# CPJKU/beat_this

Measured on AMD Instinct MI355X. Metric: audio-seconds processed/sec, higher is better.
Workload: dtype f32 activations, f16x3 products (3 x f16 MFMA on hi+lo operand halves, f32 accumulate); main-layer attention P.V: 2 x, probabilities as fp16 hi parts

## Files before the change

### beat_this_amd/csrc/gemm3.hip

```cpp
#include <cstdlib>

#include "common.h"
#include "kernels.h"

struct G3CfgS { static constexpr int BM = 128, BN = 128, BK = 32, WGM = 2, WGN = 2, NST = 3, OCC = 3; };
struct G3CfgB { static constexpr int BM = 256, BN = 256, BK = 64, WGM = 2, WGN = 4, NST = 2, OCC = 1; };
struct G3CfgT { static constexpr int BM = 192, BN = 256, BK = 64, WGM = 2, WGN = 4, NST = 2, OCC = 1; };
struct G3CfgSX { static constexpr int BM = 128, BN = 128, BK = 64, WGM = 2, WGN = 2, NST = 2, OCC = 2; };
struct G3CfgBX { static constexpr int BM = 256, BN = 256, BK = 64, WGM = 2, WGN = 4, NST = 2, OCC = 1; };
struct G3CfgTX { static constexpr int BM = 192, BN = 256, BK = 64, WGM = 2, WGN = 4, NST = 2, OCC = 1; };
struct G3CfgMX { static constexpr int BM = 256, BN = 128, BK = 32, WGM = 2, WGN = 2, NST = 3, OCC = 2; };
struct G3CfgHX { static constexpr int BM = 64, BN = 128, BK = 64, WGM = 2, WGN = 2, NST = 3, OCC = 2; };

#ifndef X3_NSPLIT
#define X3_NSPLIT 2
#endif

namespace {

typedef G3CfgS CfgS;
typedef G3CfgB CfgB;

constexpr unsigned OOB = 0x80000000u;

#ifndef BT_NT_STORE
#define BT_NT_STORE 1
#endif
#if BT_NT_STORE
#define ST_STREAM(ptr, val) __builtin_nontemporal_store((val), (ptr))
#else
#define ST_STREAM(ptr, val) (*(ptr) = (val))
#endif

typedef __amdgpu_buffer_rsrc_t rsrc_t;
typedef __attribute__((address_space(3))) void* lptr_t;
typedef __attribute__((ext_vector_type(4))) unsigned int u32x4;
typedef __attribute__((ext_vector_type(2))) unsigned int u32x2;

DEVI unsigned pk2(float a, float b) {
  const hfx2 t = {(hf)a, (hf)b};
  return __builtin_bit_cast(unsigned, t);
}

DEVI void pack_row_hf(const float (&v)[16], u32x4 (&piece)[2]) {
#pragma unroll
  for (int k = 0; k < 2; ++k) {
    unsigned x0 = pk2(v[8 * k], v[8 * k + 1]), x1 = pk2(v[8 * k + 2], v[8 * k + 3]);
    unsigned y0 = pk2(v[8 * k + 4], v[8 * k + 5]), y1 = pk2(v[8 * k + 6], v[8 * k + 7]);
    auto r0 = __builtin_amdgcn_permlane32_swap(x0, y0, false, false);
    auto r1 = __builtin_amdgcn_permlane32_swap(x1, y1, false, false);
    piece[k] = u32x4{r0[0], r1[0], r0[1], r1[1]};
  }
}

DEVI void split2(float a, float b, unsigned& whi, unsigned& wlo, float& amax) {
  split_hl(a, b, whi, wlo);
  amax = fmaxf(amax, fmaxf(fabsf(a), fabsf(b)));
}
DEVI void pack_row_hl(const float (&v)[16], u32x4 (&hi)[2], u32x4 (&lo)[2], float& amax) {
#pragma unroll
  for (int k = 0; k < 2; ++k) {
    unsigned xh[2], xl[2], yh[2], yl[2];
    split2(v[8 * k], v[8 * k + 1], xh[0], xl[0], amax);
    split2(v[8 * k + 2], v[8 * k + 3], xh[1], xl[1], amax);
    split2(v[8 * k + 4], v[8 * k + 5], yh[0], yl[0], amax);
    split2(v[8 * k + 6], v[8 * k + 7], yh[1], yl[1], amax);
    auto h0 = __builtin_amdgcn_permlane32_swap(xh[0], yh[0], false, false);
    auto h1 = __builtin_amdgcn_permlane32_swap(xh[1], yh[1], false, false);
    auto l0 = __builtin_amdgcn_permlane32_swap(xl[0], yl[0], false, false);
    auto l1 = __builtin_amdgcn_permlane32_swap(xl[1], yl[1], false, false);
    hi[k] = u32x4{h0[0], h1[0], h0[1], h1[1]};
    lo[k] = u32x4{l0[0], l1[0], l0[1], l1[1]};
  }
}
DEVI void pack_row_f8(const float (&v)[16], u32x4 (&hi)[2], u32x2 (&h8)[2], u32x2 (&l8)[2], float& amax) {
#pragma unroll
  for (int k = 0; k < 2; ++k) {
    unsigned xh[2], xl[2], yh[2], yl[2];
    split2(v[8 * k], v[8 * k + 1], xh[0], xl[0], amax);
    split2(v[8 * k + 2], v[8 * k + 3], xh[1], xl[1], amax);
    split2(v[8 * k + 4], v[8 * k + 5], yh[0], yl[0], amax);
    split2(v[8 * k + 6], v[8 * k + 7], yh[1], yl[1], amax);
    const unsigned x8 = pk4_f8(v[8 * k], v[8 * k + 1], v[8 * k + 2], v[8 * k + 3]);
    const unsigned y8 = pk4_f8(v[8 * k + 4], v[8 * k + 5], v[8 * k + 6], v[8 * k + 7]);
    const unsigned xl8 = lo4_f8(v[8 * k], v[8 * k + 1], v[8 * k + 2], v[8 * k + 3], xh[0], xh[1]);
    const unsigned yl8 = lo4_f8(v[8 * k + 4], v[8 * k + 5], v[8 * k + 6], v[8 * k + 7], yh[0], yh[1]);
    auto h0 = __builtin_amdgcn_permlane32_swap(xh[0], yh[0], false, false);
    auto h1 = __builtin_amdgcn_permlane32_swap(xh[1], yh[1], false, false);
    auto b8 = __builtin_amdgcn_permlane32_swap(x8, y8, false, false);
    auto c8 = __builtin_amdgcn_permlane32_swap(xl8, yl8, false, false);
    hi[k] = u32x4{h0[0], h1[0], h0[1], h1[1]};
    h8[k] = u32x2{b8[0], b8[1]};
    l8[k] = u32x2{c8[0], c8[1]};
  }
}
DEVI void flag_range(int* status, float amax, float limit = 65504.f) {
  if (status && __any(!(amax <= limit)) && (threadIdx.x & 63) == 0) atomicOr(status, 1);
}

template <int EPI, typename CFG, int X3 = 0, int ABL = 0>
__global__ __launch_bounds__(64 * CFG::WGM * CFG::WGN, (CFG::OCC * CFG::WGM * CFG::WGN + 3) / 4)
void gemm3_kernel(const Gemm3P p, int n_tiles, int total_tiles, int per_xcd, int nsplit) {
  constexpr int BM = CFG::BM, BN = CFG::BN, BK = CFG::BK, NST = CFG::NST;
  constexpr int NW = CFG::WGM * CFG::WGN, NT = 64 * NW;
  constexpr int TB = BM / CFG::WGM / 32;
  constexpr int FB = BN / CFG::WGN / 32;
  constexpr int ROWB = BK * 2;
  constexpr int KR = X3 ? BK / 2 : BK;
  constexpr bool HL16 = X3 && BK == 32;
  constexpr int EB = X3 ? 4 : 2;
  constexpr int CPR = ROWB / 16;
  constexpr int RPI = 64 / CPR;
  constexpr int A_BYTES = BM * ROWB, W_BYTES = BN * ROWB, ST_BYTES = A_BYTES + W_BYTES;
  constexpr int APC = A_BYTES / (NT * 16), WPC = W_BYTES / (NT * 16);
  static_assert(EPI != G3_QKV || TB == FB, "the V columns swap the operand roles: square wave tile needed");
  static_assert(BN / CFG::WGN == 64, "ssq partials are per 64 columns = one wave");
  static_assert(!X3 || ROWB == 128 || ROWB == 64, "hl32: a k-step is a whole group (128 B per row) or half of one (64 B)");
  static_assert(X3 != 2 || ROWB == 128, "hl8: a k-step is a whole 32-column group");
  static_assert(NST * ST_BYTES >= NW * 8192, "the epilogues stage 8 KB per wave in the ring's LDS");
  __shared__ __attribute__((aligned(16))) char smem[NST * ST_BYTES];
  const int bid = blockIdx.x;
  int m_tile, n_tile;
  if (nsplit <= 1) {
    const int tile = (bid & 7) * per_xcd + (bid >> 3);
    if (tile >= total_tiles) return;
    m_tile = tile / n_tiles;
    n_tile = tile - m_tile * n_tiles;
  } else {
    const int xcd = bid & 7, slot = bid >> 3;
    const int g = xcd % nsplit, j = xcd / nsplit, per_m = 8 / nsplit, nt = n_tiles / nsplit;
    const int m_local = slot / nt;
    m_tile = m_local * per_m + j;
    n_tile = g * nt + (slot - m_local * nt);
    if ((long)m_tile * n_tiles >= total_tiles) return;
  }
  const int m0 = m_tile * BM, n0 = n_tile * BN;
  const int tid = threadIdx.x, lane = tid & 63, wave = __builtin_amdgcn_readfirstlane(tid >> 6);
  const int g = lane >> 5, lr = lane & 31;
  const int wm = wave / CFG::WGN, wn = wave % CFG::WGN;
  const int nk = p.K / KR;
  auto swz = [](int r) { return ROWB == 64 ? (r >> 2) & 3 : (r >> 1) & 7; };
  const int Lv = p.nblk * 32;

  int kind = 0;
  if constexpr (EPI == G3_QKV) kind = n0 < 3 * p.inner ? n0 / p.inner : 3;
  const bool normal = EPI == G3_QKV && kind == 2;

  const unsigned a_bytes = (unsigned)((long)p.M * p.lda * EB), w_bytes = (unsigned)((long)n_tiles * BN * p.K * EB);
  static_assert(APC >= 1 && WPC >= 1, "tile too small for the workgroup");
  static_assert(APC <= 4 && WPC <= 4, "voffA / voffW hold at most 4 pieces");
  unsigned voffA[4], voffW[4];
  int tapmask[4] = {0, 0, 0, 0};
#pragma unroll
  for (int i = 0; i < APC; ++i) {
    const int r = (i * NW + wave) * RPI + lane / CPR;
    const int c = (lane % CPR) ^ swz(r);
    long row = (long)m0 + r;
    bool ok = row < p.M;
    if constexpr (EPI == G3_QKV) {
      const int seq = (int)(row / Lv), t = (int)(row - (long)seq * Lv);
      ok = seq < p.n_seq && t < p.L;
      row = (long)seq * p.L + t;
    }
#ifdef BT_ABL_HID_WRAP
    if (EPI == G3_RESID && X3 && p.K >= 1024 && p.conv_C2 == 0) row &= BT_ABL_HID_WRAP - 1;
#endif
    voffA[i] = ok ? (unsigned)(row * p.lda * EB + (HL16 ? (c >> 1) * 64 + (c & 1) * 16 : c * 16)) : OOB;
    if constexpr (EPI == G3_RESID) {
      const int t = p.conv_C2 > 0 ? (int)((row / p.conv_F) % p.conv_T) : 1;
      tapmask[i] = ok ? ((t >= 1 ? 1 : 0) | 2 | (t + 1 < p.conv_T ? 4 : 0)) : 0;
    }
  }
#pragma unroll
  for (int i = 0; i < WPC; ++i) {
    const int r = (i * NW + wave) * RPI + lane / CPR;
    const int c = (lane % CPR) ^ swz(r);
    voffW[i] = (unsigned)((long)(n0 + r) * p.K * EB + (HL16 ? (c >> 1) * 64 + (c & 1) * 16 : c * 16));
  }
  const bool conv = EPI == G3_RESID && p.conv_C2 > 0;
  const unsigned tap_bytes = conv ? (unsigned)(p.conv_F * p.conv_C2 * EB) : 0u;
  const int c2_shift = conv ? __builtin_ctz((unsigned)p.conv_C2) : 0;
  const rsrc_t rA = __builtin_amdgcn_make_buffer_rsrc(const_cast<char*>(reinterpret_cast<const char*>(p.A)) - tap_bytes, 0,
                                                      a_bytes + 2 * tap_bytes, 0x00020000);
  const rsrc_t rW = __builtin_amdgcn_make_buffer_rsrc(const_cast<void*>(p.W), 0, w_bytes, 0x00020000);
#define G3_ISSUE(kt, stage)                                                                                          \
  do {                                                                                                                \
    char* st_ = smem + (stage) * ST_BYTES + wave * 1024;                                                              \
    const int so_ = HL16 ? ((kt) >> 1) * 128 + ((kt) & 1) * 32 : (kt) * ROWB;                                         \
    if (conv) {                                                                                                       \
      const int tap_ = ((kt) * KR) >> c2_shift;                                                                       \
      const int kin_ = ((kt) * KR) & (p.conv_C2 - 1);                                                                 \
      const int soa_ = tap_ * (int)tap_bytes + (HL16 ? (kin_ >> 5) * 128 + ((kin_ >> 4) & 1) * 32 : kin_ * EB);      \
      _Pragma("unroll") for (int i_ = 0; i_ < APC; ++i_)                                                              \
          __builtin_amdgcn_raw_ptr_buffer_load_lds(rA, (lptr_t)(st_ + i_ * NW * 1024), 16,                            \
                                                   ((tapmask[i_] >> tap_) & 1) ? voffA[i_] : OOB, soa_, 0, 0);        \
    } else {                                                                                                          \
      _Pragma("unroll") for (int i_ = 0; i_ < APC; ++i_)                                                              \
          __builtin_amdgcn_raw_ptr_buffer_load_lds(rA, (lptr_t)(st_ + i_ * NW * 1024), 16, voffA[i_], so_, 0, 0);     \
    }                                                                                                                 \
    _Pragma("unroll") for (int i_ = 0; i_ < WPC; ++i_)                                                                \
        __builtin_amdgcn_raw_ptr_buffer_load_lds(rW, (lptr_t)(st_ + A_BYTES + i_ * NW * 1024), 16, voffW[i_], so_, 0, 0); \
  } while (0)

  constexpr int NP = FB, NQ = TB;
  const int pofs = (normal ? wm * (TB * 32) * ROWB : A_BYTES + wn * (FB * 32) * ROWB) + lr * ROWB;
  const int qofs = (normal ? A_BYTES + wn * (FB * 32) * ROWB : wm * (TB * 32) * ROWB) + lr * ROWB;
  const int sw = swz(lr);
  constexpr int MS = ROWB / 32;
  int kc[MS];
#pragma unroll
  for (int m = 0; m < MS; ++m) kc[m] = ((2 * m + g) ^ sw) * 16;

  f32x16 acc[NP][NQ];
#pragma unroll
  for (int a = 0; a < NP; ++a)
#pragma unroll
    for (int b = 0; b < NQ; ++b)
#pragma unroll
      for (int r = 0; r < 16; ++r) acc[a][b][r] = 0.f;

  const int row0 = m0 + wm * (TB * 32);
  long trow[TB];
  int tseq[TB], tblk[TB];
#pragma unroll
  for (int j = 0; j < TB; ++j) {
    const long v = (long)row0 + 32 * j + lr;
    if constexpr (EPI == G3_QKV) {
      const int vb = row0 + 32 * j;
      tseq[j] = vb / Lv;
      tblk[j] = (vb - tseq[j] * Lv) >> 5;
      const int t = tblk[j] * 32 + lr;
      trow[j] = (tseq[j] < p.n_seq && t < p.L) ? (long)tseq[j] * p.L + t : -1;
    } else {
      tseq[j] = tblk[j] = 0;
      trow[j] = v < p.M ? v : -1;
    }
  }
  float rs[TB], part[TB][8];
#pragma unroll
  for (int j = 0; j < TB; ++j) {
    rs[j] = 1.f;
#pragma unroll
    for (int q = 0; q < 8; ++q)
      part[j][q] = (EPI != G3_RESID && p.ssq_in && trow[j] >= 0 && q < p.ssq_parts) ? p.ssq_in[(long)q * p.M + trow[j]] : 0.f;
  }
  f32x4 bqv[EPI == G3_FF1 ? FB : 1][4];
  if constexpr (EPI == G3_FF1) {
#pragma unroll
    for (int a = 0; a < FB; ++a)
#pragma unroll
      for (int q = 0; q < 4; ++q) bqv[a][q] = *reinterpret_cast<const f32x4*>(p.bias + n0 + wn * 64 + a * 32 + 8 * q + 4 * g);
  }
  f32x4 csv[EPI == G3_QKV ? TB : 1][4];
  if constexpr (EPI == G3_QKV) {
    if (kind < 2) {
#pragma unroll
      for (int b = 0; b < TB; ++b)
#pragma unroll
        for (int q = 0; q < 4; ++q)
          csv[b][q] = tseq[b] < p.n_seq ? *reinterpret_cast<const f32x4*>(p.rope + ((long)(tblk[b] * 32 + lr) * 16 + 4 * q + 2 * g) * 2)
                                        : f32x4{0.f, 0.f, 0.f, 0.f};
    }
  }
  constexpr int LPS = APC + WPC;
#pragma unroll
  for (int s0 = 0; s0 < NST - 1; ++s0)
    if (s0 < nk) G3_ISSUE(s0, s0);
  if (EPI == G3_FF1 || EPI == G3_QKV || (EPI != G3_RESID && p.ssq_in)) {
    asm volatile("s_waitcnt vmcnt(0)" ::: "memory");
    __builtin_amdgcn_sched_barrier(0);
  }
  if (EPI != G3_RESID && p.ssq_in) {
#pragma unroll
    for (int j = 0; j < TB; ++j) {
      float sum = 0.f;
#pragma unroll
      for (int q = 0; q < 8; ++q) sum += part[j][q];
      for (int q = 8; q < p.ssq_parts; ++q) sum += trow[j] >= 0 ? p.ssq_in[(long)q * p.M + trow[j]] : 0.f;
      rs[j] = trow[j] >= 0 ? sqrtf((float)p.K) / fmaxf(sqrtf(sum), 1e-12f) : 0.f;
    }
  }
  int stage = 0, stage2 = NST - 1;
  long long t_wait = 0, t_bar = 0, t_loop0 = 0;
  if constexpr ((ABL & 8) != 0) t_loop0 = clock64();
  for (int kt = 0; kt < nk; ++kt) {
    long long tq0 = 0, tq1 = 0;
    if constexpr ((ABL & 8) != 0) tq0 = clock64();
    if (NST > 2 && kt + 1 < nk && !(ABL & 1)) asm volatile("s_waitcnt vmcnt(%0) lgkmcnt(0)" ::"n"((NST - 2) * LPS) : "memory");
    else asm volatile("s_waitcnt vmcnt(0) lgkmcnt(0)" ::: "memory");
    if constexpr ((ABL & 8) != 0) tq1 = clock64();
    __builtin_amdgcn_s_barrier();
    if constexpr ((ABL & 8) != 0) { const long long tq2 = clock64(); t_wait += tq1 - tq0; t_bar += tq2 - tq1; }
    if (kt + NST - 1 < nk && !(ABL & 1)) G3_ISSUE(kt + NST - 1, stage2);
    const char* st = smem + stage * ST_BYTES;
    if constexpr (X3 == 2) {
      typedef __attribute__((ext_vector_type(8))) int i32x8;
      const int cP = 4 + 2 * g, cQ = 6 - 2 * g;
      const int kP0 = (cP ^ sw) * 16, kP1 = ((cP + 1) ^ sw) * 16, kQ0 = (cQ ^ sw) * 16, kQ1 = ((cQ + 1) ^ sw) * 16;
      {
        i32x8 p8[NP], q8[NQ];
#pragma unroll
        for (int a = 0; a < NP; ++a) {
          const u32x4 lo = *reinterpret_cast<const u32x4*>(st + pofs + a * 32 * ROWB + kP0);
          const u32x4 hi = *reinterpret_cast<const u32x4*>(st + pofs + a * 32 * ROWB + kP1);
          p8[a] = i32x8{(int)lo[0], (int)lo[1], (int)lo[2], (int)lo[3], (int)hi[0], (int)hi[1], (int)hi[2], (int)hi[3]};
        }
#pragma unroll
        for (int b = 0; b < NQ; ++b) {
          const u32x4 lo = *reinterpret_cast<const u32x4*>(st + qofs + b * 32 * ROWB + kQ0);
          const u32x4 hi = *reinterpret_cast<const u32x4*>(st + qofs + b * 32 * ROWB + kQ1);
          q8[b] = i32x8{(int)lo[0], (int)lo[1], (int)lo[2], (int)lo[3], (int)hi[0], (int)hi[1], (int)hi[2], (int)hi[3]};
        }
#pragma unroll
        for (int a = 0; a < NP; ++a)
#pragma unroll
          for (int b = 0; b < NQ; ++b)
            acc[a][b] = __builtin_amdgcn_mfma_scale_f32_32x32x64_f8f6f4(p8[a], q8[b], acc[a][b], 0, 0, 0, HL8_SCALE_WORD, 0, 0x7f7f7f7f);
      }
#pragma unroll
      for (int m = 0; m < 2; ++m) {
        hfx8 ph[NP], qh[NQ];
#pragma unroll
        for (int a = 0; a < NP; ++a) ph[a] = *reinterpret_cast<const hfx8*>(st + pofs + a * 32 * ROWB + kc[m]);
#pragma unroll
        for (int b = 0; b < NQ; ++b) qh[b] = *reinterpret_cast<const hfx8*>(st + qofs + b * 32 * ROWB + kc[m]);
#pragma unroll
        for (int a = 0; a < NP; ++a)
#pragma unroll
          for (int b = 0; b < NQ; ++b) acc[a][b] = MFMA32_H(ph[a], qh[b], acc[a][b]);
      }
    } else if constexpr (!X3) {
#pragma unroll
      for (int m = 0; m < ((ABL & 4) ? 0 : MS); ++m) {
        hfx8 fp[NP], fq[NQ];
#pragma unroll
        for (int a = 0; a < NP; ++a) fp[a] = *reinterpret_cast<const hfx8*>(st + pofs + a * 32 * ROWB + kc[m]);
#pragma unroll
        for (int b = 0; b < NQ; ++b) fq[b] = *reinterpret_cast<const hfx8*>(st + qofs + b * 32 * ROWB + kc[m]);
#pragma unroll
        for (int a = 0; a < NP; ++a)
#pragma unroll
          for (int b = 0; b < NQ; ++b) acc[a][b] = MFMA32_H(fp[a], fq[b], acc[a][b]);
      }
    } else {
#pragma unroll
      for (int m = 0; m < ((ABL & 4) ? 0 : MS / 2); ++m) {
        hfx8 ph[NP], pl[NP], qh[NQ], ql[NQ];
#pragma unroll
        for (int a = 0; a < NP; ++a) {
          ph[a] = *reinterpret_cast<const hfx8*>(st + pofs + a * 32 * ROWB + kc[m]);
          pl[a] = *reinterpret_cast<const hfx8*>(st + pofs + a * 32 * ROWB + kc[m + MS / 2]);
        }
#pragma unroll
        for (int b = 0; b < NQ; ++b) {
          qh[b] = *reinterpret_cast<const hfx8*>(st + qofs + b * 32 * ROWB + kc[m]);
          ql[b] = *reinterpret_cast<const hfx8*>(st + qofs + b * 32 * ROWB + kc[m + MS / 2]);
        }
#pragma unroll
        for (int a = 0; a < NP; ++a)
#pragma unroll
          for (int b = 0; b < NQ; ++b) acc[a][b] = MFMA32_H(pl[a], qh[b], acc[a][b]);
#pragma unroll
        for (int a = 0; a < NP; ++a)
#pragma unroll
          for (int b = 0; b < NQ; ++b) acc[a][b] = MFMA32_H(ph[a], ql[b], acc[a][b]);
#pragma unroll
        for (int a = 0; a < NP; ++a)
#pragma unroll
          for (int b = 0; b < NQ; ++b) acc[a][b] = MFMA32_H(ph[a], qh[b], acc[a][b]);
      }
    }
    stage = stage == NST - 1 ? 0 : stage + 1;
    stage2 = stage2 == NST - 1 ? 0 : stage2 + 1;
  }

#undef G3_ISSUE
  long long t_loop1 = 0;
  if constexpr ((ABL & 8) != 0) t_loop1 = clock64();
  __syncthreads();
  char* wst = smem + wave * 8192;
  float amax = 0.f;
  if constexpr (EPI == G3_FF1 && X3) {
    char* out8 = reinterpret_cast<char*>(p.out);
    const int nb0 = n0 + wn * 64;
    const int r4 = lane >> 4, cp = lane & 15;
#pragma unroll
    for (int b = 0; b < TB; ++b) {
#pragma unroll
      for (int a = 0; a < FB; ++a) {
        float v[16];
#pragma unroll
        for (int r = 0; r < 16; ++r) v[r] = gelu_erf(fmaf(acc[a][b][r], rs[b], bqv[a][r >> 2][r & 3]));
        if (p.x3 & G3_X3_OUT_F8) {
          u32x4 hi[2];
          u32x2 h8[2], l8[2];
          pack_row_f8(v, hi, h8, l8, amax);
#pragma unroll
          for (int k = 0; k < 2; ++k) {
            *reinterpret_cast<u32x4*>(wst + lr * 256 + (((8 * a + 2 * k + g) ^ (lr & 15)) << 4)) = hi[k];
            *reinterpret_cast<u32x2*>(wst + lr * 256 + (((8 * a + 4 + k) ^ (lr & 15)) << 4) + 8 * g) = h8[k];
            *reinterpret_cast<u32x2*>(wst + lr * 256 + (((8 * a + 6 + k) ^ (lr & 15)) << 4) + 8 * g) = l8[k];
          }
        } else {
        u32x4 hi[2], lo[2];
        pack_row_hl(v, hi, lo, amax);
#pragma unroll
        for (int k = 0; k < 2; ++k) {
          *reinterpret_cast<u32x4*>(wst + lr * 256 + (((8 * a + 2 * k + g) ^ (lr & 15)) << 4)) = hi[k];
          *reinterpret_cast<u32x4*>(wst + lr * 256 + (((8 * a + 4 + 2 * k + g) ^ (lr & 15)) << 4)) = lo[k];
        }
        }
      }
      static_assert(FB == 2, "row = 64 features = 256 B of hl32");
#pragma unroll
      for (int ps = 0; ps < 8; ++ps) {
        const int r = ps * 4 + r4;
        const u32x4 w = *reinterpret_cast<const u32x4*>(wst + r * 256 + (cp << 4));
        const long row = (long)row0 + 32 * b + r;
#ifdef BT_ABL_HID_WRAP
        if (row < p.M) *reinterpret_cast<u32x4*>(out8 + ((row & (BT_ABL_HID_WRAP - 1)) * p.ldo + nb0) * 4 + ((cp ^ (r & 15)) << 4)) = w;
#else
        if (row < p.M) ST_STREAM(reinterpret_cast<u32x4*>(out8 + (row * p.ldo + nb0) * 4 + ((cp ^ (r & 15)) << 4)), w);
#endif
      }
    }
  } else if constexpr (EPI == G3_FF1) {
    hf* out = reinterpret_cast<hf*>(p.out);
    const int nb0 = n0 + wn * 64;
#pragma unroll
    for (int b = 0; b < TB; ++b) {
#pragma unroll
      for (int a = 0; a < FB; ++a) {
        float v[16];
#pragma unroll
        for (int r = 0; r < 16; ++r) {
          const float u = fmaf(acc[a][b][r], rs[b], bqv[a][r >> 2][r & 3]);
          v[r] = (ABL & 2) ? u : gelu_tanh(u);
        }
        u32x4 piece[2];
        pack_row_hf(v, piece);
#pragma unroll
        for (int k = 0; k < 2; ++k)
          *reinterpret_cast<u32x4*>(wst + lr * 128 + (((4 * a + 2 * k + g) ^ (lr & 7)) << 4)) = piece[k];
      }
      static_assert(FB == 2, "row = 64 features = 128 B");
#pragma unroll
      for (int ps = 0; ps < 4; ++ps) {
        const int r = ps * 8 + (lane >> 3), cp = lane & 7;
        const u32x4 w = *reinterpret_cast<const u32x4*>(wst + r * 128 + (cp << 4));
        const long row = (long)row0 + 32 * b + r;
        if (row < p.M) *reinterpret_cast<u32x4*>(out + row * p.ldo + nb0 + ((cp ^ (r & 7)) << 3)) = w;
      }
    }
  } else if constexpr (EPI == G3_RESID) {
    hf* xb = reinterpret_cast<hf*>(p.xb);
    const int nb0 = n0 + wn * 64;
    if (nb0 < p.N) {
    if (p.bias) {
#pragma unroll
      for (int a = 0; a < FB; ++a)
#pragma unroll
        for (int q = 0; q < 4; ++q) {
          const f32x4 bb = *reinterpret_cast<const f32x4*>(p.bias + nb0 + a * 32 + 8 * q + 4 * g);
#pragma unroll
          for (int b = 0; b < TB; ++b)
#pragma unroll
            for (int i = 0; i < 4; ++i) acc[a][b][4 * q + i] += bb[i];
        }
    }
    const int r4 = lane >> 4, cp = lane & 15;
    const unsigned ldx = (unsigned)p.ldx;
    const unsigned off_lane = (unsigned)(row0 + r4) * ldx + (unsigned)nb0;
    unsigned colq[4];
#pragma unroll
    for (int q = 0; q < 4; ++q) colq[q] = (unsigned)((cp ^ (4 * q + r4)) << 2);
    const int rows_left = p.M - row0 - r4;
    if (p.gelu) {
#pragma unroll
      for (int a = 0; a < FB; ++a)
#pragma unroll
        for (int b = 0; b < TB; ++b)
#pragma unroll
          for (int r = 0; r < 16; ++r) acc[a][b][r] = X3 ? gelu_erf(acc[a][b][r]) : gelu_tanh(acc[a][b][r]);
    }
#pragma unroll
    for (int b = 0; b < TB; ++b) {
      f32x4 xv[8];
#pragma unroll
      for (int ps = 0; ps < 8; ++ps) {
        const unsigned off = off_lane + (unsigned)(32 * b + 4 * ps) * ldx + colq[ps & 3];
        xv[ps] = (32 * b + 4 * ps < rows_left && !p.no_resid && p.x) ? *reinterpret_cast<const f32x4*>(p.x + off)
                                                               : f32x4{0.f, 0.f, 0.f, 0.f};
      }
#pragma unroll
      for (int a = 0; a < FB; ++a)
#pragma unroll
        for (int q = 0; q < 4; ++q)
          *reinterpret_cast<f32x4*>(wst + lr * 256 + (((8 * a + 2 * q + g) ^ (lr & 15)) << 4)) =
              f32x4{acc[a][b][4 * q], acc[a][b][4 * q + 1], acc[a][b][4 * q + 2], acc[a][b][4 * q + 3]};
#pragma unroll
      for (int ps = 0; ps < 8; ++ps) {
        const int r = ps * 4 + r4;
        const unsigned off = off_lane + (unsigned)(32 * b + 4 * ps) * ldx + colq[ps & 3];
        const bool ok = 32 * b + 4 * ps < rows_left;
        f32x4 v = *reinterpret_cast<const f32x4*>(wst + r * 256 + (cp << 4));
#pragma unroll
        for (int i = 0; i < 4; ++i) v[i] += xv[ps][i];
        if (ok) {
          if (p.x) *reinterpret_cast<f32x4*>(p.x + off) = v;
          if constexpr (X3) {
            if (xb) {
              const unsigned f = (unsigned)nb0 + colq[ps & 3];
              unsigned wh[2], wl[2];
              split2(v[0], v[1], wh[0], wl[0], amax);
              split2(v[2], v[3], wh[1], wl[1], amax);
              hf* d = xb + (2u * off - (f & 31u));
              *reinterpret_cast<u32x2*>(d) = u32x2{wh[0], wh[1]};
              if (p.x3 & G3_X3_OUT_F8) {
                char* gb = reinterpret_cast<char*>(d) - (f & 31u);
                *reinterpret_cast<unsigned*>(gb + 64) = pk4_f8(v[0], v[1], v[2], v[3]);
                *reinterpret_cast<unsigned*>(gb + 96) = lo4_f8(v[0], v[1], v[2], v[3], wh[0], wh[1]);
              } else {
                *reinterpret_cast<u32x2*>(d + 32) = u32x2{wl[0], wl[1]};
              }
            }
          } else {
            if (xb) *reinterpret_cast<u32x2*>(xb + off) = u32x2{pk2(v[0], v[1]), pk2(v[2], v[3])};
          }
        }
        float ssq = ok ? fmaf(v[0], v[0], fmaf(v[1], v[1], fmaf(v[2], v[2], v[3] * v[3]))) : 0.f;
#pragma unroll
        for (int o = 8; o > 0; o >>= 1) ssq += __shfl_xor(ssq, o);
        if (p.ssq_out && ok && cp == 0) p.ssq_out[(unsigned)(n0 / 64 + wn) * (unsigned)p.M + (unsigned)(row0 + 32 * b + r)] = ssq;
      }
    }
    }
  } else {
    constexpr int BLK_E = X3 ? 2048 : 1024;
    if (kind < 2) {
      hf* dst = reinterpret_cast<hf*>(kind == 0 ? p.qf : p.kf);
#pragma unroll
      for (int b = 0; b < TB; ++b) {
        if (tseq[b] >= p.n_seq) continue;
        const f32x4 (&cs)[4] = csv[b];
#pragma unroll
        for (int a = 0; a < FB; ++a) {
          const int head = (n0 - kind * p.inner + wn * 64 + a * 32) >> 5;
          hf* blk = dst + (((long)tseq[b] * p.heads + head) * p.nbp + tblk[b]) * BLK_E;
#pragma unroll
          for (int q = 0; q < 4; ++q) {
            const float e0 = acc[a][b][4 * q] * rs[b], o0 = acc[a][b][4 * q + 1] * rs[b];
            const float e1 = acc[a][b][4 * q + 2] * rs[b], o1 = acc[a][b][4 * q + 3] * rs[b];
            const float r0 = e0 * cs[q][0] - o0 * cs[q][1], r1 = o0 * cs[q][0] + e0 * cs[q][1];
            const float r2 = e1 * cs[q][2] - o1 * cs[q][3], r3 = o1 * cs[q][2] + e1 * cs[q][3];
            if constexpr (X3) {
              unsigned wh[2], wl[2];
              split2(r0, r1, wh[0], wl[0], amax);
              split2(r2, r3, wh[1], wl[1], amax);
              ST_STREAM(reinterpret_cast<u32x2*>(blk + (q * 32 + lr) * 8 + 4 * g), (u32x2{wh[0], wh[1]}));
              ST_STREAM(reinterpret_cast<u32x2*>(blk + 1024 + (q * 32 + lr) * 8 + 4 * g), (u32x2{wl[0], wl[1]}));
            } else {
              *reinterpret_cast<u32x2*>(blk + (q * 32 + lr) * 8 + 4 * g) = u32x2{pk2(r0, r1), pk2(r2, r3)};
            }
          }
        }
      }
    } else if (kind == 2) {
      hf* dst = reinterpret_cast<hf*>(p.vf);
#pragma unroll
      for (int a = 0; a < TB; ++a) {
        if (tseq[a] >= p.n_seq) continue;
        float sk[16];
#pragma unroll
        for (int r = 0; r < 16; ++r) sk[r] = __shfl(rs[a], crow(r, g));
#pragma unroll
        for (int b = 0; b < FB; ++b) {
          const int head = (n0 - 2 * p.inner + wn * 64 + b * 32) >> 5;
          hf* blk = dst + (((long)tseq[a] * p.heads + head) * p.nbp + tblk[a]) * BLK_E;
#pragma unroll
          for (int s = 0; s < 2; ++s) {
            unsigned w[4], wl[4] = {0, 0, 0, 0};
#pragma unroll
            for (int i = 0; i < 4; ++i) {
              const float v0 = acc[a][b][8 * s + 2 * i] * sk[8 * s + 2 * i], v1 = acc[a][b][8 * s + 2 * i + 1] * sk[8 * s + 2 * i + 1];
              if constexpr (X3) split2(v0, v1, w[i], wl[i], amax);
              else w[i] = pk2(v0, v1);
            }
            ST_STREAM(reinterpret_cast<u32x4*>(blk + (s * 64 + lane) * 8), (u32x4{w[0], w[1], w[2], w[3]}));
            if constexpr (X3) ST_STREAM(reinterpret_cast<u32x4*>(blk + 1024 + (s * 64 + lane) * 8), (u32x4{wl[0], wl[1], wl[2], wl[3]}));
          }
        }
      }
    } else {
#pragma unroll
      for (int b = 0; b < TB; ++b) {
        if (tseq[b] >= p.n_seq) continue;
        const int t = tblk[b] * 32 + lr;
#pragma unroll
        for (int a = 0; a < FB; ++a)
#pragma unroll
          for (int r = 0; r < 16; ++r) {
            const int h = n0 - 3 * p.inner + wn * 64 + a * 32 + crow(r, g);
            if (h < p.heads)
              p.gates[((long)tseq[b] * p.heads + h) * p.nbp * 32 + t] = sigmoidf(fmaf(acc[a][b][r], rs[b], p.b_gates[h]));
          }
      }
    }
  }
  if constexpr (X3) flag_range(p.status, amax, (p.x3 & G3_X3_OUT_F8) ? HL8_ACT_MAX : 65504.f);
  if constexpr ((ABL & 8) != 0) {
    const long long t_end = clock64();
    __syncthreads();
    if (lane == 0) {
      long long* dbg = reinterpret_cast<long long*>(EPI == G3_RESID ? p.out : (void*)const_cast<float*>(p.ssq_in));
      long long* d = dbg + ((long)blockIdx.x * NW + wave) * 4;
      d[0] = t_loop1 - t_loop0; d[1] = t_wait; d[2] = t_bar; d[3] = t_end - t_loop1;
    }
  }
}

template <int EPI, typename CFG, int X3 = 0, int ABL = 0>
void launch_cfg(const Gemm3P& p, hipStream_t s) {
  const int n_tiles = (p.N + CFG::BN - 1) / CFG::BN;
  const long rows = p.epi == G3_QKV ? (long)p.n_seq * p.nblk * 32 : (long)p.M;
  const long m_tiles = (rows + CFG::BM - 1) / CFG::BM;
  const long total = m_tiles * n_tiles;
  int nsplit = (p.x3 >> 4) & 15;
  if (nsplit == 0) nsplit = (X3 && X3_NSPLIT > 1 && (long)n_tiles * CFG::BN * p.K * 4 > (5L << 19) && n_tiles % X3_NSPLIT == 0) ? X3_NSPLIT : 1;
  if (nsplit != 2 && nsplit != 4 && nsplit != 8) nsplit = 1;
  if (n_tiles % nsplit) nsplit = 1;
  long per;
  if (nsplit == 1) {
    per = (total + 7) / 8;
    per = (per + n_tiles - 1) / n_tiles * n_tiles;
  } else {
    const long per_m = 8 / nsplit;
    per = (m_tiles + per_m - 1) / per_m * (n_tiles / nsplit);
  }
  dim3 grid((unsigned)(per * 8)), block(64 * CFG::WGM * CFG::WGN);
  hipLaunchKernelGGL((gemm3_kernel<EPI, CFG, X3, ABL>), grid, block, 0, s, p, n_tiles, (int)total, (int)per, nsplit);
}

}

bool gemm3_supported(const Gemm3P& p) {
  const int eb = p.x3 ? 4 : 2;
  if (p.M <= 0 || p.K % 64 != 0 || p.K < 128 || p.lda % 8 != 0) return false;
  if ((long)p.M * p.lda * eb >= 0x7fffffffL || (long)(p.N + 255) / 256 * 256 * p.K * eb >= 0x7fffffffL) return false;
  if (p.x3 && BT_HALF_IS_BF16) return false;
  if (p.conv_C2 > 0 && (p.epi != G3_RESID || (p.conv_C2 & (p.conv_C2 - 1)) || p.conv_C2 % 32 != 0 || p.lda != p.conv_C2 ||
                        p.K != 3 * p.conv_C2 || p.conv_F <= 0 || p.conv_T <= 0 || p.M % (p.conv_T * p.conv_F) != 0 || !p.no_resid))
    return false;
  if (p.epi == G3_RESID && !p.x && !p.xb) return false;
  if (p.epi == G3_QKV) return p.inner % 128 == 0 && p.inner == p.heads * 32 && p.L > 0 && (long)p.n_seq * ((p.L + 31) / 32 * 32) < 0x7fffffffL;
  if (p.epi == G3_FF1) return p.N % 128 == 0 && p.ldo % 8 == 0;
  if (p.epi == G3_RESID) return p.N % 64 == 0 && p.ldx % 8 == 0 && (long)(p.M + 256) * p.ldx * (p.x3 ? 2 : 1) < 0x7fffffffL &&
                                (long)(p.N / 64) * p.M < 0x7fffffffL;
  return false;
}

#ifndef X3_BIG_FF1
#define X3_BIG_FF1 0
#endif
#ifndef X3_MX
#define X3_MX 1
#endif

int launch_gemm3(const Gemm3P& p, hipStream_t s) {
  if (!gemm3_supported(p)) return -2;
#ifdef BT_DEV
  static const int abl = getenv("BT_G3_ABL") ? atoi(getenv("BT_G3_ABL")) : 0;
  static const int force_big = getenv("BT_G3_BIG") ? atoi(getenv("BT_G3_BIG")) : -1;
#else
  constexpr int abl = 0, force_big = -1;
#endif
  const bool big_ok = p.epi != G3_QKV && p.N % 256 == 0;
  const int force = (p.x3 & 15) == 2 ? 1 : (p.x3 & 15) == 3 ? 0 : force_big;
  const bool forced_small = (p.x3 & 15) == 4 || (p.x3 & 15) == 5;
  const long tiles192 = ((long)p.M + 191) / 192 * (p.N / 256);
  const bool fills = !p.x3 || tiles192 >= 160;
  const bool big = big_ok && !forced_small && (force == 1 || (force != 0 && p.epi == G3_RESID && p.K >= 1024 && p.M >= 4096 && fills) ||
                              (force != 0 && p.x3 && X3_BIG_FF1 && p.epi == G3_FF1 && p.M >= 4096));
  auto cost = [&](int bm) { const long t = ((long)p.M + bm - 1) / bm * (p.N / 256); return (t + 255) / 256 * bm; };
  const bool rows192 = big && p.epi == G3_RESID && force != 1 && cost(192) < cost(256);
  const long mx_tiles = ((long)p.M + 255) / 256 * ((p.N + 127) / 128);
  const bool f8 = (p.x3 & G3_X3_F8) != 0;
  const bool mx = p.x3 && !f8 && p.epi != G3_QKV && !big && !rows192 && force != 0 &&
                  ((p.x3 & 15) == 4 || (X3_MX && mx_tiles >= 512 && p.M >= 20000));
  const long sx_tiles = ((long)p.M + 127) / 128 * ((p.N + 127) / 128);
  const bool hx = p.x3 && p.epi == G3_RESID && !big && !rows192 && !mx &&
                  ((p.x3 & 15) == 5 || ((p.x3 & 15) <= 1 && force_big < 0 && (sx_tiles < 256 || (p.K < 1024 && p.M < 20000))));
  if (p.x3) {
#ifdef BT_DEV
    if (abl == 8 && p.epi == G3_FF1) { launch_cfg<G3_FF1, G3CfgSX, true, 8>(p, s); return (int)hipGetLastError(); }
    if (abl == 1 || abl == 4) {
      const bool b = big || rows192;
      if (p.epi == G3_FF1) { if (abl == 1) { if (b) launch_cfg<G3_FF1, G3CfgBX, true, 1>(p, s); else launch_cfg<G3_FF1, G3CfgSX, true, 1>(p, s); }
                             else { if (b) launch_cfg<G3_FF1, G3CfgBX, true, 4>(p, s); else launch_cfg<G3_FF1, G3CfgSX, true, 4>(p, s); } }
      else if (p.epi == G3_RESID) { if (abl == 1) { if (b) launch_cfg<G3_RESID, G3CfgBX, true, 1>(p, s); else launch_cfg<G3_RESID, G3CfgSX, true, 1>(p, s); }
                                    else { if (b) launch_cfg<G3_RESID, G3CfgBX, true, 4>(p, s); else launch_cfg<G3_RESID, G3CfgSX, true, 4>(p, s); } }
      else { if (abl == 1) launch_cfg<G3_QKV, G3CfgSX, true, 1>(p, s); else launch_cfg<G3_QKV, G3CfgSX, true, 4>(p, s); }
      return (int)hipGetLastError();
    }
#endif
    if (f8) {
      if (p.epi == G3_QKV) launch_cfg<G3_QKV, G3CfgSX, 2>(p, s);
      else if (p.epi == G3_FF1) { if (big) launch_cfg<G3_FF1, G3CfgBX, 2>(p, s); else launch_cfg<G3_FF1, G3CfgSX, 2>(p, s); }
      else if (hx) launch_cfg<G3_RESID, G3CfgHX, 2>(p, s);
      else if (rows192) launch_cfg<G3_RESID, G3CfgTX, 2>(p, s);
      else if (big) launch_cfg<G3_RESID, G3CfgBX, 2>(p, s);
      else launch_cfg<G3_RESID, G3CfgSX, 2>(p, s);
      return (int)hipGetLastError();
    }
    switch (p.epi) {
      case G3_FF1:
        if (mx) launch_cfg<G3_FF1, G3CfgMX, true>(p, s);
        else if (big) launch_cfg<G3_FF1, G3CfgBX, true>(p, s); else launch_cfg<G3_FF1, G3CfgSX, true>(p, s);
        break;
      case G3_RESID:
        if (mx) launch_cfg<G3_RESID, G3CfgMX, true>(p, s);
        else if (hx) launch_cfg<G3_RESID, G3CfgHX, true>(p, s);
        else if (rows192) launch_cfg<G3_RESID, G3CfgTX, true>(p, s);
        else if (big) launch_cfg<G3_RESID, G3CfgBX, true>(p, s);
        else launch_cfg<G3_RESID, G3CfgSX, true>(p, s);
        break;
      case G3_QKV: launch_cfg<G3_QKV, G3CfgSX, true>(p, s); break;
      default: return -1;
    }
    return (int)hipGetLastError();
  }
  switch (p.epi) {
    case G3_FF1:
      if (big) launch_cfg<G3_FF1, CfgB>(p, s);
#ifdef BT_DEV
      else if (abl == 8) launch_cfg<G3_FF1, CfgS, false, 8>(p, s);
#endif
      else launch_cfg<G3_FF1, CfgS>(p, s);
      break;
    case G3_RESID:
#ifdef BT_DEV
      if (big && abl == 8) { launch_cfg<G3_RESID, CfgB, false, 8>(p, s); break; }
      if (!big && abl == 8) { launch_cfg<G3_RESID, CfgS, false, 8>(p, s); break; }
#endif
      if (rows192) launch_cfg<G3_RESID, G3CfgT>(p, s);
      else if (big) launch_cfg<G3_RESID, CfgB>(p, s);
      else launch_cfg<G3_RESID, CfgS>(p, s);
      break;
    case G3_QKV: launch_cfg<G3_QKV, CfgS>(p, s); break;
    default: return -1;
  }
  return (int)hipGetLastError();
}
```

### beat_this_amd/csrc/kernels.h

```cpp
#pragma once
#include <hip/hip_runtime.h>
#include <stdint.h>

#ifndef BT_PREC_F32
#define BT_PREC_F32 0
#define BT_PREC_HALF 1
#endif
#ifndef BT_PREC_F32X3
#define BT_PREC_F32X3 3
#endif

enum {
  GEMM_EPI_STORE = 0,
  GEMM_EPI_RESID = 1,
  GEMM_EPI_QKV = 2
};
enum {
  GEMM_F_RMS = 1,
  GEMM_F_BIAS = 2,
  GEMM_F_GELU = 4,
  GEMM_F_OUT_F32 = 8,
  GEMM_F_A_F32 = 16,
  GEMM_F_CONV = 32,
  GEMM_F_ROWMAP = 64
};

struct GemmP {
  const void* A;
  long lda;
  const void* W;
  int M, N, K;
  int epi, flags;
  const float* bias;
  void* out;
  long ldo;
  float* x;
  long ldx;
  void* xb;
  float* ssq_out;
  int conv_C2, conv_T, conv_F;
  float* gates;
  int inner;
  int heads;
  const float* rope;
  int pdiv, pmod;
  int map_T, map_F;
};
int launch_gemm(const GemmP& p, int prec, hipStream_t s);

enum { G3_FF1 = 0, G3_RESID = 1, G3_QKV = 2 };
struct Gemm3P {
  const void* A; long lda; int M, K;
  const void* W; int N;
  int epi;
  const float* bias;
  const float* ssq_in; int ssq_parts;
  void* out; long ldo;
  float* x; long ldx; void* xb;
  float* ssq_out;
  int n_seq, L, nblk, nbp, heads, inner;
  const float* rope; void* qf; void* kf; void* vf; float* gates; const float* b_gates;
  int no_resid;
  int gelu;
  int conv_C2, conv_T, conv_F;
  int x3;
  int* status;
};
enum { G3_X3_F8 = 0x100, G3_X3_OUT_F8 = 0x200 };
bool gemm3_supported(const Gemm3P& p);
int launch_gemm3(const Gemm3P& p, hipStream_t s);

struct GemmMx8P {
  const void* A; const void* SA;
  const void* W; const void* SW;
  float* out; long ldo;
  int M, N, K;
};
bool gemm_mx8_supported(const GemmMx8P& p);
int launch_gemm_mx8(const GemmMx8P& p, hipStream_t s);

struct AttnP {
  const void* qkv;
  long ld;
  const float* gates;
  void* out;
  int n_seq, L, heads, inner;
  int o_div;
  long o_outer, o_inner, o_tok;
};
int launch_attn_flash(const AttnP& p, int prec, hipStream_t s);

struct AttnFragP {
  const void* q; const void* k; const void* v;
  const float* gates;
  void* out;
  int n_seq, L, heads, inner, nbp;
  int o_div;
  long o_outer, o_inner, o_tok;
  int x3, out_f32;
  int* status;
  int* fix_mask;
};
int attn_frag_blocks(int L);
int launch_attn_frag(const AttnFragP& p, hipStream_t s);

struct QkvFrontP {
  const float* x;
  int B, T, F, C;
  const void* wfrag;
  const float* b_gates;
  const float* rope;
  void* q; void* k; void* v;
  float* gates;
  int nbp;
  int x3;
  int* status;
};
int launch_qkv_front(const QkvFrontP& p, hipStream_t s);

struct FusedFFP {
  float* x; long M; int C;
  const void* wfrag;
  const float* b1; const float* b2;
  void* xb;
};
int launch_ff_fused(const FusedFFP& p, int prec, hipStream_t s);

struct FusedOutFFP {
  float* x; long M; int C;
  const void* ao;
  const void* wfrag;
  const float* b1; const float* b2;
  void* xb;
  int abl;
};
int launch_outff_fused(const FusedOutFFP& p, int prec, hipStream_t s);
struct FusedAttnFFP {
  float* x; long M; int C;
  const float* b_gates; const float* rope;
  const void* wfrag;
  const float* b1; const float* b2;
};
int launch_attnff_fused(const FusedAttnFFP& p, int prec, hipStream_t s);

struct LayerTailP {
  float* x; long M; int C; int hidden;
  const void* ao;
  const void* wfrag;
  const float* b1; const float* b2;
  void* xb;
  float* ssq_out;
};
bool layer_tail_supported(int C, int hidden);
int launch_layer_tail(const LayerTailP& p, hipStream_t s);

struct StemP {
  const float* spect;
  float* x;
  const float* bn1_scale; const float* bn1_shift;
  const float* w;
  const float* bias;
  int B, T;
};
int launch_stem(const StemP& p, hipStream_t s);

struct HeadP {
  const float* x;
  const float* w;
  float b0, b1;
  float* beat; float* downbeat;
  int M, D, sum_head;
  int prenorm;
  int* status;
};
int launch_head(const HeadP& p, hipStream_t s);
int launch_clear_words(int* w, int n, hipStream_t s);
int launch_norm_out(const float* x, const float* gamma, float* y, long M, int D, hipStream_t s, int* status = nullptr);
int launch_finite_rows(const float* x, long M, int D, int* status, hipStream_t s);
int launch_shadow_ssq(const float* x, void* xb, float* ssq, long M, int D, hipStream_t s, int hl32 = 0);

struct bt_span_t { const float* data; long n; long out_off; long n_out; };

int launch_split(const float* spect, long n_frames, const int* starts, const int* table, int B, int T, float* chunks,
                 hipStream_t s, int border = 0);
int launch_aggregate(const float* cb, const float* cd, const int* starts, const int* table, const int* pieces, int n_pieces,
                     int B, int T, int border, long n_frames, float* beat, float* downbeat, hipStream_t s);
int launch_resample(const bt_span_t& one, const bt_span_t* tracks, int n_tracks, long max_n_out, int up, int down,
                    const float* h, int half, float* y, hipStream_t s);
int launch_peaks(const float* logits, long n, const int* spans, int n_arrays, int* idx, int* count, hipStream_t s);

struct LogmelP {
  bt_span_t one;
  const bt_span_t* tracks;
  int n_tracks; long max_frames;
  const float* window;
  const float* twiddle;
  const int* mel_start;
  const int* mel_len;
  const float* mel_w;
  float* spect;
};
int launch_logmel(const LogmelP& p, hipStream_t s);
```

Before: 62850.

## Prefetch residual x tiles into LDS ring during RESID GEMM epilogue

In the x3 residual-epilogue GEMM, the residual input x is now streamed into reused LDS pipeline stages with buffer_load_lds, so it is no longer read with direct global loads per block. The first block is issued during the last k-iteration when the stage layout allows it, and later blocks are refilled into the slots as they free up. This aims to hide global latency of the residual read behind the accumulator write-out and the MMA tail. It adds a new x3 mode flag that forces the 192-row config, plus a flag that keeps the old global path, and the LDS slot reuse makes waitcnt and barrier ordering more delicate.

```diff
diff --git a/beat_this_amd/csrc/gemm3.hip b/beat_this_amd/csrc/gemm3.hip
--- a/beat_this_amd/csrc/gemm3.hip
+++ b/beat_this_amd/csrc/gemm3.hip
@@ -183,7 +183,24 @@
   const rsrc_t rA = __builtin_amdgcn_make_buffer_rsrc(const_cast<char*>(reinterpret_cast<const char*>(p.A)) - tap_bytes, 0,
                                                       a_bytes + 2 * tap_bytes, 0x00020000);
   const rsrc_t rW = __builtin_amdgcn_make_buffer_rsrc(const_cast<void*>(p.W), 0, w_bytes, 0x00020000);
-#define G3_ISSUE(kt, stage)                                                                                          \
+  constexpr bool XST = EPI == G3_RESID && X3 == 1 && !(ABL & 16);
+  constexpr int XROW = NW * 8192, XS0 = NST * ST_BYTES / XROW, XS = XS0 < TB ? XS0 : TB;
+  constexpr bool XEARLY = XST && NST == 2 && ST_BYTES == XROW;
+  static_assert(!XST || XS >= 1, "the ring holds at least one x block per wave");
+  const bool has_x = XST && !p.no_resid && p.x && n0 + wn * 64 < p.N;
+  const unsigned x_lane = (unsigned)((m0 + wm * (TB * 32)) + (lane >> 4)) * (unsigned)p.ldx + (unsigned)(n0 + wn * 64);
+  const int x_left = p.M - (m0 + wm * (TB * 32)) - (lane >> 4);
+  const rsrc_t rX = __builtin_amdgcn_make_buffer_rsrc(p.x, 0, XST ? (unsigned)((long)p.M * p.ldx * 4) : 0u, 0x00020000);
+#define G3_ISSUE_X(b, slot)                                                                                           \
+  do {                                                                                                                \
+    _Pragma("unroll") for (int ps_ = 0; ps_ < 8; ++ps_) {                                                             \
+      const unsigned o_ = x_lane + (unsigned)(32 * (b) + 4 * ps_) * (unsigned)p.ldx +                                 \
+                          (unsigned)(((lane & 15) ^ (4 * (ps_ & 3) + (lane >> 4))) << 2);                             \
+      __builtin_amdgcn_raw_ptr_buffer_load_lds(rX, (lptr_t)((slot) + ps_ * 1024), 16,                                 \
+                                               32 * (b) + 4 * ps_ < x_left ? o_ * 4u : 0u, 0, 0, 0);                  \
+    }                                                                                                                 \
+  } while (0)
+#define G3_ISSUE(kt, stage)                                                                                        \
   do {                                                                                                                \
     char* st_ = smem + (stage) * ST_BYTES + wave * 1024;                                                              \
     const int so_ = HL16 ? ((kt) >> 1) * 128 + ((kt) & 1) * 32 : (kt) * ROWB;                                         \
@@ -292,6 +309,7 @@
     __builtin_amdgcn_s_barrier();
     if constexpr ((ABL & 8) != 0) { const long long tq2 = clock64(); t_wait += tq1 - tq0; t_bar += tq2 - tq1; }
     if (kt + NST - 1 < nk && !(ABL & 1)) G3_ISSUE(kt + NST - 1, stage2);
+    if constexpr (XEARLY) if (kt == nk - 1 && has_x) G3_ISSUE_X(0, smem + stage2 * ST_BYTES + wave * 8192);
     const char* st = smem + stage * ST_BYTES;
     if constexpr (X3 == 2) {
       typedef __attribute__((ext_vector_type(8))) int i32x8;
@@ -377,7 +395,8 @@
 #undef G3_ISSUE
   long long t_loop1 = 0;
   if constexpr ((ABL & 8) != 0) t_loop1 = clock64();
-  __syncthreads();
+  if constexpr (XST) asm volatile("s_waitcnt lgkmcnt(0)\n\ts_barrier" ::: "memory");
+  else __syncthreads();
   char* wst = smem + wave * 8192;
   float amax = 0.f;
   if constexpr (EPI == G3_FF1 && X3) {
@@ -456,6 +475,13 @@
     hf* xb = reinterpret_cast<hf*>(p.xb);
     const int nb0 = n0 + wn * 64;
     if (nb0 < p.N) {
+    char* xslot[XS];
+#pragma unroll
+    for (int s = 0; s < XS; ++s) xslot[s] = smem + (XEARLY ? (s == 0 ? stage : stage2) * ST_BYTES : s * XROW) + wave * 8192;
+    if (has_x) {
+#pragma unroll
+      for (int s = XEARLY ? 1 : 0; s < XS; ++s) G3_ISSUE_X(s, xslot[s]);
+    }
     if (p.bias) {
 #pragma unroll
       for (int a = 0; a < FB; ++a)
@@ -485,27 +511,46 @@
     }
 #pragma unroll
     for (int b = 0; b < TB; ++b) {
+      char* const wb = XST ? xslot[b % XS] : wst;
       f32x4 xv[8];
+      if constexpr (XST) {
+        if (has_x && (b == 0 || b >= XS)) asm volatile("s_waitcnt vmcnt(0)" ::: "memory");
+#pragma unroll
+        for (int ps = 0; ps < 8; ++ps)
+          xv[ps] = has_x ? *reinterpret_cast<const f32x4*>(wb + (ps * 4 + r4) * 256 + (cp << 4)) : f32x4{0.f, 0.f, 0.f, 0.f};
+      } else {
+#pragma unroll
+        for (int ps = 0; ps < 8; ++ps) {
+          const unsigned off = off_lane + (unsigned)(32 * b + 4 * ps) * ldx + colq[ps & 3];
+          xv[ps] = (32 * b + 4 * ps < rows_left && !p.no_resid && p.x) ? *reinterpret_cast<const f32x4*>(p.x + off)
+                                                                 : f32x4{0.f, 0.f, 0.f, 0.f};
+        }
+      }
+#pragma unroll
+      for (int a = 0; a < FB; ++a)
+#pragma unroll
+        for (int q = 0; q < 4; ++q)
+          *reinterpret_cast<f32x4*>(wb + lr * 256 + (((8 * a + 2 * q + g) ^ (lr & 15)) << 4)) =
+              f32x4{acc[a][b][4 * q], acc[a][b][4 * q + 1], acc[a][b][4 * q + 2], acc[a][b][4 * q + 3]};
 #pragma unroll
       for (int ps = 0; ps < 8; ++ps) {
-        const unsigned off = off_lane + (unsigned)(32 * b + 4 * ps) * ldx + colq[ps & 3];
-        xv[ps] = (32 * b + 4 * ps < rows_left && !p.no_resid && p.x) ? *reinterpret_cast<const f32x4*>(p.x + off)
-                                                               : f32x4{0.f, 0.f, 0.f, 0.f};
-      }
-#pragma unroll
-      for (int a = 0; a < FB; ++a)
-#pragma unroll
-        for (int q = 0; q < 4; ++q)
-          *reinterpret_cast<f32x4*>(wst + lr * 256 + (((8 * a + 2 * q + g) ^ (lr & 15)) << 4)) =
-              f32x4{acc[a][b][4 * q], acc[a][b][4 * q + 1], acc[a][b][4 * q + 2], acc[a][b][4 * q + 3]};
+        f32x4 v = *reinterpret_cast<const f32x4*>(wb + (ps * 4 + r4) * 256 + (cp << 4));
+#pragma unroll
+        for (int i = 0; i < 4; ++i) v[i] += xv[ps][i];
+        xv[ps] = v;
+      }
+      if constexpr (XST) {
+        if (has_x && b + XS < TB) {
+          asm volatile("s_waitcnt lgkmcnt(0)" ::: "memory");
+          G3_ISSUE_X(b + XS, wb);
+        }
+      }
 #pragma unroll
       for (int ps = 0; ps < 8; ++ps) {
         const int r = ps * 4 + r4;
         const unsigned off = off_lane + (unsigned)(32 * b + 4 * ps) * ldx + colq[ps & 3];
         const bool ok = 32 * b + 4 * ps < rows_left;
-        f32x4 v = *reinterpret_cast<const f32x4*>(wst + r * 256 + (cp << 4));
-#pragma unroll
-        for (int i = 0; i < 4; ++i) v[i] += xv[ps][i];
+        const f32x4 v = xv[ps];
         if (ok) {
           if (p.x) *reinterpret_cast<f32x4*>(p.x + off) = v;
           if constexpr (X3) {
@@ -607,6 +652,7 @@
       }
     }
   }
+#undef G3_ISSUE_X
   if constexpr (X3) flag_range(p.status, amax, (p.x3 & G3_X3_OUT_F8) ? HL8_ACT_MAX : 65504.f);
   if constexpr ((ABL & 8) != 0) {
     const long long t_end = clock64();
@@ -640,6 +686,11 @@
   dim3 grid((unsigned)(per * 8)), block(64 * CFG::WGM * CFG::WGN);
   hipLaunchKernelGGL((gemm3_kernel<EPI, CFG, X3, ABL>), grid, block, 0, s, p, n_tiles, (int)total, (int)per, nsplit);
 }
+template <typename CFG>
+void launch_resid_x3(const Gemm3P& p, hipStream_t s) {
+  if (p.x3 & G3_X3_X_GLOBAL) launch_cfg<G3_RESID, CFG, true, 16>(p, s);
+  else launch_cfg<G3_RESID, CFG, true>(p, s);
+}
 
 }
 
@@ -675,14 +726,15 @@
   constexpr int abl = 0, force_big = -1;
 #endif
   const bool big_ok = p.epi != G3_QKV && p.N % 256 == 0;
-  const int force = (p.x3 & 15) == 2 ? 1 : (p.x3 & 15) == 3 ? 0 : force_big;
+  const bool forced_tx = (p.x3 & 15) == 6 && p.epi == G3_RESID;
+  const int force = (p.x3 & 15) == 2 || forced_tx ? 1 : (p.x3 & 15) == 3 ? 0 : force_big;
   const bool forced_small = (p.x3 & 15) == 4 || (p.x3 & 15) == 5;
   const long tiles192 = ((long)p.M + 191) / 192 * (p.N / 256);
   const bool fills = !p.x3 || tiles192 >= 160;
   const bool big = big_ok && !forced_small && (force == 1 || (force != 0 && p.epi == G3_RESID && p.K >= 1024 && p.M >= 4096 && fills) ||
                               (force != 0 && p.x3 && X3_BIG_FF1 && p.epi == G3_FF1 && p.M >= 4096));
   auto cost = [&](int bm) { const long t = ((long)p.M + bm - 1) / bm * (p.N / 256); return (t + 255) / 256 * bm; };
-  const bool rows192 = big && p.epi == G3_RESID && force != 1 && cost(192) < cost(256);
+  const bool rows192 = big && p.epi == G3_RESID && (forced_tx || (force != 1 && cost(192) < cost(256)));
   const long mx_tiles = ((long)p.M + 255) / 256 * ((p.N + 127) / 128);
   const bool f8 = (p.x3 & G3_X3_F8) != 0;
   const bool mx = p.x3 && !f8 && p.epi != G3_QKV && !big && !rows192 && force != 0 &&
@@ -718,11 +770,11 @@
         else if (big) launch_cfg<G3_FF1, G3CfgBX, true>(p, s); else launch_cfg<G3_FF1, G3CfgSX, true>(p, s);
         break;
       case G3_RESID:
-        if (mx) launch_cfg<G3_RESID, G3CfgMX, true>(p, s);
-        else if (hx) launch_cfg<G3_RESID, G3CfgHX, true>(p, s);
-        else if (rows192) launch_cfg<G3_RESID, G3CfgTX, true>(p, s);
-        else if (big) launch_cfg<G3_RESID, G3CfgBX, true>(p, s);
-        else launch_cfg<G3_RESID, G3CfgSX, true>(p, s);
+        if (mx) launch_resid_x3<G3CfgMX>(p, s);
+        else if (hx) launch_resid_x3<G3CfgHX>(p, s);
+        else if (rows192) launch_resid_x3<G3CfgTX>(p, s);
+        else if (big) launch_resid_x3<G3CfgBX>(p, s);
+        else launch_resid_x3<G3CfgSX>(p, s);
         break;
       case G3_QKV: launch_cfg<G3_QKV, G3CfgSX, true>(p, s); break;
       default: return -1;
diff --git a/beat_this_amd/csrc/kernels.h b/beat_this_amd/csrc/kernels.h
--- a/beat_this_amd/csrc/kernels.h
+++ b/beat_this_amd/csrc/kernels.h
@@ -66,7 +66,7 @@
   int x3;
   int* status;
 };
-enum { G3_X3_F8 = 0x100, G3_X3_OUT_F8 = 0x200 };
+enum { G3_X3_F8 = 0x100, G3_X3_OUT_F8 = 0x200, G3_X3_X_GLOBAL = 0x400 };
 bool gemm3_supported(const Gemm3P& p);
 int launch_gemm3(const Gemm3P& p, hipStream_t s);
 
```

Result: no change. 62880 (median of 6 runs) (+0.1%).
